# 10XGenomics/lariat

Measured on AMD Instinct MI355X. Metric: read-pairs/sec aligned to hg38 (per-barcode align loop: SMEM seeding + SW + RFA/MAPQ on device); synthetic hg38-scale reference, higher is better.
Workload: dtype u64/i32 (FM-index + integer DP), f64 (RFA scores)

## Files before the change

lariat_amd/csrc/k_rfa.h:

```cpp
#pragma once
#include "k_aln.h"

struct DInf {
    uint8_t *active, *is_proper, *bwa_pick, *active_molecule, *duplicate;
    int32_t *molecule_id, *mapq;
    double *mol_diff, *mol_conf, *sum_move;
    i64* mate;
    int32_t* cand_read;
    i64 *active_idx, *second_best_idx, *split_idx;
    double *second_best_score, *as_score, *split_second_best, *split_score;
    int32_t* split_mapq;
};

#ifdef LH_EMU
static const u64 lh_go_cooked[607] = {
#include "go_rng_cooked.inc"
};
static const uint32_t lh_go_lpow[1848] = {
#include "go_rng_lehmer_pow.inc"
};
#else
__device__ const u64 lh_go_cooked[607] = {
#include "go_rng_cooked.inc"
};
// ... 97 lines not shown
    i64 cs = -1, ce = -1;
    if (R.rid[a] >= 0 && cen_start[R.rid[a]] >= 0) { cs = cen_start[R.rid[a]]; ce = cen_end[R.rid[a]]; }
    return R.pos[a] > cs && R.pos[a] <= ce;
}

struct RfaTab {
    int32_t* plist;
    int32_t* molraw;
    int32_t* mstart;
    int32_t* newid;
    int32_t* nreads;
    double* sval;
    int32_t* seen_rid;
    int32_t* ccnt;
    int32_t* coff;
    int32_t* kidx;
    int32_t* molc;
    int32_t* ppos;
    int32_t* rdl;
    int32_t* firstf;
    int32_t* actc;
    int32_t* psum;
    int32_t* seg0;
    int32_t* seg1;
    int32_t* nbest;
    int32_t* aoff;
    int32_t* alen;
    int32_t* act_store;
    int32_t* act_cand;
    int32_t* act_slot;
    int32_t* tdel;
    int32_t* tset;
    int32_t* mflag;
    double* P;
    u64 *dk0, *dk1, *dk2, *dk3;
    int32_t* htab;
    int32_t* gstk;
    i64* spl;
    int32_t* bestT;
};
template <typename I> struct RfaHot {
    I *nbest, *aoff, *alen, *mflag;
    I *act_store;
    I *act_cand, *act_slot, *tdel, *tset;
    double* P;
};
#ifndef LH_RFA_SM_NR
#define LH_RFA_SM_NR 256
#endif
#ifndef LH_RFA_SM_NC
#define LH_RFA_SM_NC 512
#endif
#ifndef LH_RFA_SM_M
#define LH_RFA_SM_M 128
#endif
static_assert(LH_RFA_SM_NR < 32768 && LH_RFA_SM_NC < 32768 && LH_RFA_SM_M < 32768 && LH_RFA_SM_NR % 4 == 0 && LH_RFA_SM_NC % 4 == 0 && LH_RFA_SM_M % 4 == 0, "the small instance's tables are signed 16-bit words, each array 8-byte aligned");
template <int SMALL> struct RfaHotWord { typedef int32_t type; };
template <> struct RfaHotWord<1> { typedef int16_t type; };
#define RFA_HOT_OFF (16 * LH_RFA_SRC_CHUNK)
#define RFA_HOT_BYTES (8 * LH_RFA_SM_M + 2 * (4 * LH_RFA_SM_M + LH_RFA_SM_NC + 4 * LH_RFA_SM_NR))
#define RFA_T_MASK 0x3fffffff
#define RFA_T_PAIR 0x40000000

__device__ __forceinline__ int dev_mol_active(int alen, int nbest, int change) {
    double active = (double)(alen + change), potential = (double)nbest;
    if (active <= 4) return 0;
    if (active / potential < 0.1) return 0;
    return 1;
}

#define LH_SPLIT_MAX 64
#ifndef LH_RFA_SORT_LDS
#define LH_RFA_SORT_LDS 768
#endif
#define LH_RFA_LDS_BYTES (LH_RFA_SORT_LDS * 12)

static_assert(LH_RFA_LDS_BYTES >= LH_MAPQ_TOP * 64 * (int)sizeof(double), "estimateMapQualities keeps a read's top-15 scores per lane in lds_raw (top[k * 64 + lane])");
#define LH_RFA_NCONT_LDS 1024
#define LH_RFA_SRC_CHUNK 256
static_assert(RFA_HOT_OFF + RFA_HOT_BYTES <= LH_RFA_LDS_BYTES && LH_RFA_SM_NR <= LH_RFA_SRC_CHUNK && LH_RFA_SM_NC <= LH_RFA_SORT_LDS,
              "the small instance: hot tables behind the staging of a whole source (at most a barcode's reads), every contig list sorted in LDS");
#ifndef LH_RFA_MOL_LDS_MIN
#ifndef LH_RFA_TIE_LDS
#define LH_RFA_TIE_LDS (LH_RFA_LDS_BYTES / 4 < 4096 ? LH_RFA_LDS_BYTES / 4 : 4096)
#endif
#ifndef LH_RFA_NET_BLOCK
#define LH_RFA_NET_BLOCK 1024
#endif
static_assert(LH_RFA_NET_BLOCK >= 64 && (LH_RFA_NET_BLOCK & (LH_RFA_NET_BLOCK - 1)) == 0 && LH_RFA_NET_BLOCK * 8 <= LH_RFA_LDS_BYTES, "the network's block lives in lds_raw");
#define LH_RFA_MOL_LDS_MIN 24
#endif

template <typename HOT>
__device__ __forceinline__ double dev_fast_score_w(const DCand& R, const DInf& S, const RfaTab& T, const HOT& H, i64 c_lo, int r0, int M, int src, int snk, double lup,
                                                   int32_t* sLr, int32_t* sFl, double* sLap, int* num_out, int record, int* nmove, int staged = 0) {
    const int lane = LANE();
    double change = 0, alignment_change = 0;
    int num = 0, nm = 0;
    const int n = H.alen[src], ao = H.aoff[src];
    const int reuse = staged && n <= LH_RFA_SRC_CHUNK;
    for (int cb = 0; cb < n; cb += LH_RFA_SRC_CHUNK) {
        int cn = n - cb < LH_RFA_SRC_CHUNK ? n - cb : LH_RFA_SRC_CHUNK;
        if (!reuse) {
            EMU_SYNC();
            for (int s = lane; s < cn; s += 64) {
                int a = H.act_store[ao + cb + s];
                int lr = S.cand_read[c_lo + a] - r0;
                int sm = H.act_cand[lr ^ 1];
                int hm = sm >= 0 && S.molecule_id[c_lo + sm] == src;
                int hp = hm && dev_is_pair(R, c_lo + a, c_lo + sm);
                sLr[s] = lr; sFl[s] = hm | hp << 1; sLap[s] = R.lap[c_lo + a];
            }
            WAVE_SYNC();
        }
        if (snk >= 0) {
            for (int s0 = 0; s0 < cn; s0 += 4) {
                int tq4[4];
                double lap4[4];
#pragma unroll
                for (int u = 0; u < 4; ++u) tq4[u] = s0 + u < cn ? T.bestT[(size_t)sLr[s0 + u] * M + snk] : -1;
#pragma unroll
                for (int u = 0; u < 4; ++u) lap4[u] = tq4[u] >= 0 ? R.lap[c_lo + (tq4[u] & RFA_T_MASK)] : 0.0;
#pragma unroll
                for (int u = 0; u < 4; ++u) {
                    const int tq = tq4[u], s = s0 + u;
                    if (tq >= 0) {
                        int t = tq & RFA_T_MASK, fl = sFl[s];
                        int hm = fl & 1, hp = fl >> 1;
                        int skp = (tq & RFA_T_PAIR) && hm;
                        if (!hp || (hm && skp)) {
                            if (record) { H.tdel[nm] = sLr[s]; H.tset[nm] = t; }
                            nm++;
                        }
                        alignment_change += lap4[u] - sLap[s];
                        if (hp && !skp) alignment_change += lup / 2.0;
                        else if (!hp && skp) alignment_change -= lup / 2.0;
                        num++;
                    }
                }
            }
        }
    }
    if (snk >= 0) {
        int sb = dev_mol_active(H.alen[src], H.nbest[src], 0), sa = dev_mol_active(H.alen[src], H.nbest[src], -num);
        if (!sa && sb) change -= (double)H.nbest[src] * -0.5;
        int kb = dev_mol_active(H.alen[snk], H.nbest[snk], 0), ka = dev_mol_active(H.alen[snk], H.nbest[snk], num);
        if (ka && !kb) change += (double)H.nbest[snk] * -0.5;
        if (H.alen[src] - num == 0 && num > 0) change -= -3.0;
        if (H.alen[snk] == 0 && num > 0) change += -3.0;
        change += alignment_change;
    }
    *num_out = num;
    if (nmove) *nmove = nm;
    return change;
}

__device__ __forceinline__ u64 dev_mix64(u64 x) {
    x ^= x >> 33; x *= 0xff51afd7ed558ccdull; x ^= x >> 33; x *= 0xc4ceb9fe1a85ec53ull; x ^= x >> 33;
    return x;
}

__device__ __forceinline__ void dev_tag_pair_serial(const DCand& R, const DInf& S, double improper, u64 seed, int p, int nA, int nM, u64* ring) {
    const int ra = 2 * p, rb = 2 * p + 1;
    DGoRng rng;
    dev_go_seed(rng, seed, ring);
    double best = -1.7976931348623157e308;
    i64 ba = -1, bm = -1;
    for (i64 a = R.cand_off[ra]; a < R.cand_off[ra + 1]; ++a) {
        if (!R.in_filtered[a]) continue;
        for (i64 m = R.cand_off[rb]; m < R.cand_off[rb + 1]; ++m) {
            if (!R.in_filtered[m]) continue;
            double total = dev_score_aln(R, S, improper, a, m, 0.0) + (dev_go_f64(rng) / 2.0);
            if (total > best) { best = total; ba = a; bm = m; }
        }
    }
    S.active[ba] = 1; S.bwa_pick[ba] = 1;
    if (dev_is_pair(R, ba, bm)) { S.is_proper[ba] = 1; S.is_proper[bm] = 1; }
    S.active[bm] = 1; S.bwa_pick[bm] = 1;
    (void)nA; (void)nM;
}
#ifndef LH_RFA_TAG_WAVE
#define LH_RFA_TAG_WAVE 128
#define LH_RFA_MAPQ_WAVE 128
#define LH_RFA_MQ_CHUNK 384
#endif
static_assert(24 * LH_RFA_MQ_CHUNK <= LH_RFA_LDS_BYTES, "mate staging of estimateMapQualities");


__global__ void __launch_bounds__(256) k_rfa_init(int n_reads, DCand R, DInf S, i64 cand_cap) {
    const i64 n_cand = R.cand_off[n_reads] < cand_cap ? R.cand_off[n_reads] : cand_cap;
    for (i64 g = (i64)blockIdx.x * blockDim.x + threadIdx.x; g < n_cand; g += (i64)gridDim.x * blockDim.x) {
        S.active[g] = 0; S.is_proper[g] = 0; S.bwa_pick[g] = 0; S.active_molecule[g] = 0; S.duplicate[g] = 0; S.molecule_id[g] = -1; S.mapq[g] = 0;
        S.mol_diff[g] = 0; S.mol_conf[g] = 0.00075 * 0.025; S.sum_move[g] = 1.0; S.mate[g] = -1;
    }
    for (i64 r = (i64)blockIdx.x * blockDim.x + threadIdx.x; r < n_reads; r += (i64)gridDim.x * blockDim.x) {
        S.active_idx[r] = -1; S.second_best_idx[r] = -1; S.split_idx[r] = -1; S.second_best_score[r] = 0; S.as_score[r] = 0;
        S.split_second_best[r] = 0; S.split_score[r] = 0; S.split_mapq[r] = 0;
    }
}
__global__ void __launch_bounds__(256) k_rfa_tag(DOpts o, int n_pairs, const u64* __restrict__ name_seed, DCand R, DInf S, i64 cand_cap, int32_t* __restrict__ hp_list,
                                                  int32_t* __restrict__ hp_count) {
    static_assert(LH_RFA_TAG_WAVE <= LH_GO_FAST_DRAWS, "a light pair's draws come from the state-free generator");
    const int p = blockIdx.x * blockDim.x + threadIdx.x, lane = LANE();
    int hv = 0;
    if (p < n_pairs && R.cand_off[2 * p + 2] <= cand_cap) {
        for (int h = 0; h < 2; ++h) {
            const i64 c0 = R.cand_off[2 * p + h];
            if (R.cand_off[2 * p + h + 1] - c0 == 1 && S.cand_read[c0] < 0) S.cand_read[c0] = 2 * p + h;
        }
        int nA = 0, nM = 0;
        for (i64 a = R.cand_off[2 * p]; a < R.cand_off[2 * p + 1]; ++a) nA += R.in_filtered[a] != 0;
        for (i64 m = R.cand_off[2 * p + 1]; m < R.cand_off[2 * p + 2]; ++m) nM += R.in_filtered[m] != 0;
        hv = (i64)nA * nM > LH_RFA_TAG_WAVE;
        if (!hv) dev_tag_pair_serial(R, S, o.improper_pair_penalty, name_seed[p], p, nA, nM, (u64*)nullptr);
    }
    const u64 mh = __ballot(hv);
    if (mh) {
        int basep = 0;
        if (lane == 0) basep = atomicAdd(hp_count, (int32_t)__popcll(mh));
        basep = wave_readlane(basep, 0);
        if (hv) hp_list[basep + lanes_below(mh, lane)] = p;
    }
}
__global__ void __launch_bounds__(64) k_rfa_tag_w(DOpts o, const u64* __restrict__ name_seed, DCand R, DInf S, uint8_t* __restrict__ slab_pool, i64 slab_bytes,
                                                   const int32_t* __restrict__ hp_list, const int32_t* __restrict__ hp_count, int32_t* __restrict__ status) {
    __shared__ __attribute__((aligned(16))) uint8_t lds_raw[8 * 1024];
    const int lane = LANE();
    uint8_t* slab = slab_pool + (size_t)blockIdx.x * (size_t)slab_bytes;
    const double improper = o.improper_pair_penalty;
    const int n_items = *hp_count;
    for (int item = blockIdx.x; item < n_items; item += gridDim.x) {
            const int p = hp_list[item];
            WAVE_SYNC();
            if ((size_t)(R.cand_off[2 * p + 2] - R.cand_off[2 * p]) * 12 + 16 > (size_t)slab_bytes || LH_GO_RING_BYTES > (size_t)slab_bytes) {
                if (lane == 0) status[2 * p] |= LH_ST_POOL_OVERFLOW;
                continue;
            }
            const i64 c_lo = R.cand_off[2 * p];
            const i64 a0 = R.cand_off[2 * p], a1 = R.cand_off[2 * p + 1], m1 = R.cand_off[2 * p + 2];
            int32_t* const fa = (int32_t*)slab;
            double* const fs = (double*)(slab + (((size_t)(m1 - a0) * 4 + 7) & ~(size_t)7));
            int nA = 0, nM = 0;
            for (int side = 0; side < 2; ++side) {
                const i64 lo = side ? a1 : a0, hi = side ? m1 : a1;
                int cnt = 0;
                for (i64 cb = lo; cb < hi; cb += 64) {
                    const i64 c = cb + lane;
                    const int ok = c < hi && R.in_filtered[c];
                    const u64 mk = __ballot(ok);
                    if (ok) {
                        double sc = (double)(R.mismatches[c] * -2 + R.indels[c] * -3);
                        if (R.soft_clipped[c] > 0) { sc -= 5.0 * (double)R.soft_clipped[c]; sc -= (double)R.soft_clipped_length[c] * 0.5; }
                        const int at = nA + cnt + lanes_below(mk, lane);
                        fa[at] = (int32_t)(c - c_lo); fs[at] = sc;
                    }
                    cnt += __popcll(mk);
                }
                if (side) nM = cnt; else nA = cnt;
            }
            WAVE_SYNC();
            u64* const xb = (u64*)lds_raw;
            i64 sd = (i64)name_seed[p] % 2147483647ll;
            if (sd < 0) sd += 2147483647ll;
            if (sd == 0) sd = 89482311;
            const uint32_t x0 = (uint32_t)sd;
            const i64 K = (i64)nA * nM;
            double best = -1.7976931348623157e308;
            i64 bk = 0x7fffffffffffffffll;
            int redraw = 0;
            for (i64 k0 = 0; k0 < K; k0 += 64) {
                const i64 k = k0 + lane, n = k + 1;
                const u64 va = n > LH_GO_LEN ? xb[(n - LH_GO_LEN) & 1023] : dev_go_vec0(x0, (int)(n <= 334 ? 334 - n : 941 - n));
                const u64 vb = n > LH_GO_TAP ? xb[(n - LH_GO_TAP) & 1023] : dev_go_vec0(x0, (int)(LH_GO_LEN - n));
                const u64 x = va + vb;
                xb[n & 1023] = x;
                if (k < K) {
                    const double f = (double)(i64)(x & 0x7fffffffffffffffull) * (1.0 / 9223372036854775808.0);
                    redraw |= f == 1.0;
                    const int ia = (int)(k / nM), im = (int)(k - (i64)ia * nM);
                    const i64 a = c_lo + fa[ia], m = c_lo + fa[nA + im];
                    double t = fs[ia] + fs[nA + im];
                    if (!dev_is_pair(R, a, m)) t += improper;
                    t += 0.0;
                    const double total = t + f / 2.0;
                    if (total > best) { best = total; bk = k; }
                }
                WAVE_SYNC();
            }
            if (__any(redraw)) {
                if (lane == 0) dev_tag_pair_serial(R, S, improper, name_seed[p], p, nA, nM, (u64*)slab + lane);
                WAVE_SYNC();
                continue;
            }
            for (int msk = 32; msk >= 1; msk >>= 1) {
                const double ob = __shfl_xor(best, msk);
                const i64 ok = shfl_xor_i64(bk, msk);
                if (ob > best || (ob == best && ok < bk)) { best = ob; bk = ok; }
            }
            if (lane == 0) {
                const i64 ba = c_lo + fa[(int)(bk / nM)], bm = c_lo + fa[nA + (int)(bk % nM)];
                S.active[ba] = 1; S.bwa_pick[ba] = 1;
                if (dev_is_pair(R, ba, bm)) { S.is_proper[ba] = 1; S.is_proper[bm] = 1; }
                S.active[bm] = 1; S.bwa_pick[bm] = 1;
            }
            WAVE_SYNC();
    }
// ... 600 lines not shown
                                    if (t0 > 0) { best = T.sval[i]; found = T.psum[i]; first = T.firstf[i]; }
                                    scan_tile(A, lr, lrm, arev, 0, tn, t0, e, bp, bi, first);
                                    if (bp != S2_NONE || bi != S2_NONE) { found = 1; const double x = best_of(bp, bi); if (x > best) best = x; }
                                    if (t0 + tn >= msz) { T.sval[i] = found ? best : R.lap[c_lo + T.plist[i]]; T.firstf[i] = first; }
                                    else { T.sval[i] = best; T.psum[i] = found; T.firstf[i] = first; }
                                }
                            }
                        }
                        i0 += msz;
                        continue;
                    }
                    int i1 = NCf;
                    if (i0 + ME_CAP < NCf) i1 = T.mstart[T.molraw[i0 + ME_CAP]];
                    const int tn = i1 - i0;
                    WAVE_SYNC();
                    for (int j = lane; j < tn; j += 64) { const MEnt E = load_ent(i0 + j); me[j] = E; mrd[j] = (uint16_t)(E.rd & 0xffffu); }
                    WAVE_SYNC();
                    RFA_PROF(17)
                    for (int e0 = 0; e0 < tn; e0 += 64) {
                        const int e = e0 + lane;
                        if (e < tn) {
                            const int i = i0 + e, m = T.molraw[i];
                            const int j0 = T.mstart[m] - i0, j1 = T.mstart[m + 1] - i0;
                            const MEnt A = me[e];
                            const int lr = (int)(A.rd & 0x7fffffffu), lrm = lr ^ 1, arev = (int)(A.rd >> 31);
                            int first = 1, bp = S2_NONE, bi = S2_NONE;
                            scan_tile(A, lr, lrm, arev, j0, j1, 0, e, bp, bi, first);
                            T.sval[i] = bp != S2_NONE || bi != S2_NONE ? best_of(bp, bi) : R.lap[c_lo + T.plist[i]];
                            T.firstf[i] = first;
                        }
                    }
                    RFA_PROF(18)
                    i0 = i1;
                }
                WAVE_SYNC();
            }
            int nfirst = 0, nactive = 0;
            for (int base = 0; base < NCf; base += 64) {
                int i = base + lane, first = 0, isact = 0;
                const int pre = i < NCf ? T.firstf[i] : -1;
                if (i < NCf && pre >= 0) { first = pre; isact = S.active[c_lo + T.plist[i]] != 0; }
                u64 mf = __ballot(first), ma = __ballot(isact);
                if (i < NCf) { T.psum[i] = nfirst + lanes_below(mf, lane); T.actc[i] = nactive + lanes_below(ma, lane); }
                nfirst += __popcll(mf); nactive += __popcll(ma);
            }
            if (lane == 0) { T.psum[NCf] = nfirst; T.actc[NCf] = nactive; }
            WAVE_SYNC();
            RFA_PROF(5)
            RFA_FENCE()
            int ao = 0;
            for (int base = 0; base < Mraw; base += 64) {
                int m = base + lane;
                int keep = m < Mraw && T.actc[T.mstart[m + 1]] - T.actc[T.mstart[m]] > 0;
                int nr = keep ? T.psum[T.mstart[m + 1]] - T.psum[T.mstart[m]] : 0;
                u64 mk = __ballot(keep);
                int id = M + lanes_below(mk, lane);
                int inc = wave_scan_add_i32(nr);
                if (keep) {
                    T.newid[m] = id; T.seg0[id] = T.mstart[m]; T.seg1[id] = T.mstart[m + 1];
                    if (!SMALL || id < LH_RFA_SM_M) { H.nbest[id] = nr; H.aoff[id] = ao + inc - nr; H.alen[id] = 0; }
                }
                else if (m < Mraw) T.newid[m] = -1;
                M += __popcll(mk);
                ao += wave_readlane(inc, 63);
            }
            WAVE_SYNC();
            if (SMALL && M > LH_RFA_SM_M) RFA_OVERFLOW()
            if ((size_t)M * (size_t)nR > best_cap) RFA_OVERFLOW()
            for (size_t x = lane; x < (size_t)M * nR; x += 64) T.bestT[x] = -1;
            for (int r = lane; r < nR; r += 64) { H.act_cand[r] = -1; H.act_slot[r] = -1; T.dk0[r] = 0; }
            for (int i = lane; i < NCf; i += 64) S.molecule_id[c_lo + T.plist[i]] = T.newid[T.molraw[i]];
            WAVE_SYNC();
            int nact = 0;
            for (int base = 0; base < NCf; base += 64) {
                int i = base + lane;
                int m = -1, isf = 0, act = -1;
                if (i < NCf) { m = T.newid[T.molraw[i]]; isf = T.firstf[i] && m >= 0; }
                if (isf) {
                    int mr = T.molraw[i], g = r0 + T.rdl[i];
                    double best = -1.7976931348623157e308;
                    int bi = -1, bpos = 0x7fffffff, apos = -1;
                    const i64 cb0 = R.cand_off[g], cb1 = R.cand_off[g + 1];
                    for (i64 b4 = cb0; b4 < cb1; b4 += 4) {
                        int mm[4], pj[4], ac[4];
                        double sv4[4];
#pragma unroll
                        for (int u = 0; u < 4; ++u) {
                            const int ok = b4 + u < cb1;
                            const int lb = (int)(b4 + u - c_lo);
                            mm[u] = ok ? T.molc[lb] : -2; pj[u] = ok ? T.ppos[lb] : 0; ac[u] = ok ? (int)S.active[b4 + u] : 0;
                        }
#pragma unroll
                        for (int u = 0; u < 4; ++u) sv4[u] = mm[u] == mr ? T.sval[pj[u]] : 0.0;
#pragma unroll
                        for (int u = 0; u < 4; ++u) {
                            if (mm[u] != mr) continue;
                            const int lb = (int)(b4 + u - c_lo), j = pj[u];
                            const double sv = sv4[u];
                            if (sv > best || (sv == best && j < bpos)) { best = sv; bi = lb; bpos = j; }
                            if (ac[u] && j > apos) { apos = j; act = lb; }
                        }
                    }
                    T.bestT[(size_t)T.rdl[i] * M + m] = bi;
                    atomicOr((unsigned long long*)&T.dk0[T.rdl[i]], 1ull << ((m >> 6) & 63));
                }
                int hasact = isf && act >= 0;
                u64 mk = __ballot(hasact);
                if (i < NCf) { T.actc[i] = hasact ? act : -1; T.psum[i] = nact + lanes_below(mk, lane); }
                nact += __popcll(mk);
            }
            if (lane == 0) T.psum[NCf] = nact;
            WAVE_SYNC();
            for (int i = lane; i < NCf; i += 64) {
                int m = T.newid[T.molraw[i]];
                if (m < 0 || !T.firstf[i]) continue;
                int lr = T.rdl[i];
                int t = T.bestT[(size_t)lr * M + m] & RFA_T_MASK, tm = T.bestT[(size_t)(lr ^ 1) * M + m];
                if (tm >= 0 && dev_is_pair(R, c_lo + t, c_lo + (tm & RFA_T_MASK))) T.bestT[(size_t)lr * M + m] = t | RFA_T_PAIR;
                int act = T.actc[i];
                if (act >= 0) {
                    int slot = T.psum[i] - T.psum[T.seg0[m]];
                    H.act_store[H.aoff[m] + slot] = act; H.act_cand[lr] = act; H.act_slot[lr] = slot;
                }
            }
            for (int m = lane; m < M; m += 64) H.alen[m] = T.psum[T.seg1[m]] - T.psum[T.seg0[m]];
            WAVE_SYNC();
            for (int m = lane; m < M; m += 64) {
                int diffs = 0;
                for (int k = 0; k < H.alen[m]; ++k) diffs += R.mismatches[c_lo + H.act_store[H.aoff[m] + k]];
                double diff = (double)diffs / (double)H.alen[m];
                for (int k = 0; k < H.alen[m]; ++k) S.mol_diff[c_lo + H.act_store[H.aoff[m] + k]] = diff;
            }
            WAVE_SYNC();
            RFA_PROF(6)
            RFA_FENCE()
            auto stage_source = [&](int src) -> u64 {
                if (M <= 64 || H.alen[src] > LH_RFA_SRC_CHUNK) return ~0ull;
                int num;
                dev_fast_score_w(R, S, T, H, c_lo, r0, M, src, -1, improper, sLr, sFl, sLap, &num, 0, (int*)0);
                u64 mine = 0;
                for (int k = lane; k < H.alen[src]; k += 64) mine |= T.dk0[sLr[k]];
                u64 all = 0;
                for (int b = 0; b < 64 && b * 64 < M; ++b)
                    if (__ballot((int)(mine >> b & 1))) all |= 1ull << b;
                if (M > 64 * 64) all = ~0ull;
                return all;
            };
            int source = 0, idle = 0;
            for (int it = 0; it < 8 * M && idle < M; ++it) {
                ++idle;
                if (H.alen[source] == 0) { source = (source + 1) % M; continue; }
                double bs = -1.7976931348623157e308;
                int bl = -1, bi = 0x7fffffff;
                const u64 groups = stage_source(source);
                const int staged = groups != ~0ull;
                for (int sb = 0; sb < M; sb += 64) {
                    if (!(groups >> ((sb >> 6) & 63) & 1)) continue;
                    int i = sb + lane, num;
                    int snk = (i < M && i != source) ? i : -1;
                    double sc = dev_fast_score_w(R, S, T, H, c_lo, r0, M, source, snk, improper, sLr, sFl, sLap, &num, 0, (int*)0, staged);
                    if (snk >= 0 && num > 0 && (sc > bs || (sc == bs && H.alen[i] > bl))) { bs = sc; bl = H.alen[i]; bi = i; }
                }
                for (int msk = 32; msk >= 1; msk >>= 1) {
                    double os = __shfl_xor(bs, msk);
                    int ol = __shfl_xor(bl, msk), oi = __shfl_xor(bi, msk);
                    int take = oi != 0x7fffffff && (bi == 0x7fffffff || os > bs || (os == bs && (ol > bl || (ol == bl && oi < bi))));
                    if (take) { bs = os; bl = ol; bi = oi; }
                }
                if (bi != 0x7fffffff && (bs > 0 || (bs == 0 && bl > H.alen[source]))) {
                    int num, nmv;
                    dev_fast_score_w(R, S, T, H, c_lo, r0, M, source, bi, improper, sLr, sFl, sLap, &num, lane == 0, &nmv, staged);
                    WAVE_SYNC();
                    idle = 0;
                    if (lane == 0) {
                        for (int k = 0; k < nmv; ++k) {
                            int lr = H.tdel[k], t = H.tset[k];
                            int a = H.act_cand[lr], slot = H.act_slot[lr];
                            int last = H.alen[source] - 1;
                            if (H.alen[source] > 1) {
                                int mv = H.act_store[H.aoff[source] + last];
                                H.act_store[H.aoff[source] + slot] = mv;
                                H.act_slot[S.cand_read[c_lo + mv] - r0] = slot;
                            }
                            H.alen[source] = last;
                            H.act_store[H.aoff[bi] + H.alen[bi]] = t;
                            H.act_slot[lr] = H.alen[bi]; H.act_cand[lr] = t;
                            H.alen[bi]++;
                            S.active[c_lo + a] = 0; S.active[c_lo + t] = 1;
                        }
                    }
                }
                WAVE_SYNC();
                source = (source + 1) % M;
            }
            RFA_PROF(7)
            RFA_FENCE()
            for (int s = 0; s < M; ++s) {
                const u64 groups = stage_source(s);
                const int staged = groups != ~0ull;
                for (int sb = 0; sb < M; sb += 64) {
                    if (!(groups >> ((sb >> 6) & 63) & 1)) continue;
                    int t = sb + lane, num;
                    double sc = dev_fast_score_w(R, S, T, H, c_lo, r0, M, s, (t < M && t != s) ? t : -1, improper, sLr, sFl, sLap, &num, 0, (int*)0, staged);
                    if (t < M) H.P[t] = t == s ? 0.0 : pow(10.0, sc);
                }
                WAVE_SYNC();
                RFA_PROF(8)
                for (int k = lane; k < H.alen[s]; k += 64) {
                    int a = H.act_store[H.aoff[s] + k], lr = S.cand_read[c_lo + a] - r0;
                    double sum = S.sum_move[c_lo + a];
                    const u64 mine = M > 64 && M <= 64 * 64 ? T.dk0[lr] : ~0ull;
                    for (int t0 = 0; t0 < M; t0 += 8) {
                        if (!(mine >> ((t0 >> 6) & 63) & 1)) { t0 = (t0 | 63) - 7; continue; }
                        int q8[8];
#pragma unroll
                        for (int u = 0; u < 8; ++u) q8[u] = t0 + u < M ? T.bestT[(size_t)lr * M + t0 + u] : -1;
#pragma unroll
                        for (int u = 0; u < 8; ++u)
                            if (t0 + u != s && q8[u] >= 0) sum += H.P[t0 + u];
                    }
                    S.sum_move[c_lo + a] = sum;
                }
                WAVE_SYNC();
                RFA_PROF(2)
            }
            RFA_PROF(8)
            RFA_FENCE()
            for (int m = lane; m < M; m += 64) {
                double conf = (double)H.alen[m] / (double)H.nbest[m];
                int soft = 0, diffs = 0;
                for (int k = 0; k < H.alen[m]; ++k) {
                    int a = H.act_store[H.aoff[m] + k];
                    if (R.soft_clipped[c_lo + a] > 0) soft++;
                    diffs += R.mismatches[c_lo + a];
                }
                double diff = (double)diffs / (double)H.alen[m];
                for (int k = 0; k < H.alen[m]; ++k) {
                    int a = H.act_store[H.aoff[m] + k];
                    S.mol_conf[c_lo + a] = conf; S.mol_diff[c_lo + a] = diff;
                }
                H.mflag[m] = (H.alen[m] - soft > 4 && conf > 0.1) ? 1 : 0;
            }
            WAVE_SYNC();
            for (int i = lane; i < NCf; i += 64) {
                int a = T.plist[i], m = S.molecule_id[c_lo + a];
                if (m != -1) S.active_molecule[c_lo + a] = (uint8_t)H.mflag[m];
            }
            WAVE_SYNC();
        }
        {
            double part = 0.0;
            if (do_rfa && M > 0) {
                for (int m = 0; m < M; ++m) {
                    const int al = H.alen[m], ao = H.aoff[m];
                    if (H.mflag[m]) {
                        i64 smallest = 0x7fffffffffffffffll, biggest = -1;
                        for (int k = lane; k < al; k += 64) {
                            i64 p = R.pos[c_lo + H.act_store[ao + k]];
                            if (p > biggest) biggest = p;
                            if (p < smallest) smallest = p;
                        }
                        for (int msk = 32; msk >= 1; msk >>= 1) {
                            const i64 ob = shfl_xor_i64(biggest, msk), os = shfl_xor_i64(smallest, msk);
                            if (ob > biggest) biggest = ob;
                            if (os < smallest) smallest = os;
                        }
                        if (lane == 0 && biggest >= smallest) part += (double)(biggest - smallest) + 1000.0;
                    } else {
                        for (int k = lane; k < al; k += 64) {
                            i64 g = c_lo + H.act_store[ao + k];
                            part += (double)(R.aend[g] - R.pos[g]) * 2.0;
                        }
                    }
                }
            }
            for (int msk = 32; msk >= 1; msk >>= 1) part += __shfl_xor(part, msk);
            if (lane == 0) shd[0] = (do_rfa && M > 0) ? log10((1000.0 + part) / o.genome_length * 0.05) : 0.0;
        }
        WAVE_SYNC();
        double lmp = shd[0];
        RFA_PROF(9)
        RFA_FENCE()
        for (int r = lane; r < nR; r += 64) {
            i64 act = -1;
            for (i64 a = R.cand_off[r0 + r]; a < R.cand_off[r0 + r + 1]; ++a) if (R.in_filtered[a] && S.active[a]) act = a;
            S.active_idx[r0 + r] = act;
        }
        WAVE_SYNC();
        for (int r = lane; r < nR; r += 64) {
            i64 a = S.active_idx[r0 + r], m = S.active_idx[r0 + (r ^ 1)];
            S.mate[a] = m;
        }
        WAVE_SYNC();
        if (lane == 0) bc_lmp[bc] = lmp;
        for (int rb_ = 0; rb_ < nR; rb_ += 64) {
            const int r = rb_ + lane;
            int hv = 0;
            if (r < nR) hv = (R.cand_off[r0 + r + 1] - R.cand_off[r0 + r]) * (R.cand_off[r0 + (r ^ 1) + 1] - R.cand_off[r0 + (r ^ 1)]) > LH_RFA_MAPQ_WAVE;
            const u64 mh = __ballot(hv);
            if (mh) {
                int basep = 0;
                if (lane == 0) basep = atomicAdd(hr_count, (int32_t)__popcll(mh));
                basep = wave_readlane(basep, 0);
                if (hv) { const int at = basep + lanes_below(mh, lane); hr_list[2 * at] = r0 + r; hr_list[2 * at + 1] = bc; }
            }
        }
        WAVE_SYNC();
        RFA_PROF(10)
        RFA_FENCE()
        for (int r = lane; r < nR; r += 64) {
            int gr = r0 + r, gm = r0 + (r ^ 1);
            i64 a0 = R.cand_off[gr], a1 = R.cand_off[gr + 1], m0 = R.cand_off[gm], m1 = R.cand_off[gm + 1];
            if ((a1 - a0) * (m1 - m0) > LH_RFA_MAPQ_WAVE) continue;
            double* const top = (double*)lds_raw;
#define TOPV(k_) top[(k_) * 64 + lane]
            int ntop = 0;
#define TOP_PUSH(v_)                                                                   \
    {                                                                                  \
        double v = (v_);                                                               \
        int k_ = ntop < LH_MAPQ_TOP ? ntop : LH_MAPQ_TOP;                              \
        if (ntop < LH_MAPQ_TOP || v > TOPV(LH_MAPQ_TOP - 1)) {                         \
            if (ntop < LH_MAPQ_TOP) ntop++; else k_ = LH_MAPQ_TOP - 1;                 \
            while (k_ > 0 && TOPV(k_ - 1) < v) { TOPV(k_) = TOPV(k_ - 1); k_--; }      \
            TOPV(k_) = v;                                                              \
        }                                                                              \
    }
            i64 first = -1;
            for (i64 a = a0; a < a1; ++a) if (R.in_filtered[a]) { first = a; break; }
            double bestSingle = -1.7976931348623157e308;
            for (i64 m = m0; m < m1; ++m) {
                if (!R.in_filtered[m]) continue;
                double s = dev_score_aln(R, S, improper, -1, m, lmp);
                if (s > bestSingle) bestSingle = s;
            }
            double pseudo = bestSingle + dev_pseudo_score(R, first, lmp);
            TOP_PUSH(pseudo)
            for (i64 a = a0; a < a1; ++a) {
                if (!R.in_filtered[a]) continue;
                double best = -1.7976931348623157e308;
                for (i64 m = m0; m < m1; ++m) {
                    if (!R.in_filtered[m]) continue;
                    double s = dev_score_aln(R, S, improper, a, m, lmp);
                    if (s > best) best = s;
                }
                TOP_PUSH(best)
            }
            double sb_raw = pseudo, sb_lp = -1000.0;
            i64 sb_aln = -1;
            for (i64 a = a0; a < a1; ++a) {
                if (!R.in_filtered[a] || S.active[a]) continue;
                for (i64 m = m0; m < m1; ++m) {
                    if (!R.in_filtered[m]) continue;
                    double s = dev_score_aln(R, S, improper, a, m, lmp);
                    if (s > sb_lp) { sb_lp = s; sb_raw = dev_score_aln(R, S, improper, a, m, 0.0); sb_aln = a; S.mate[a] = m; }
                }
            }
            i64 act = S.active_idx[gr];
            S.second_best_idx[gr] = sb_aln; S.second_best_score[gr] = sb_raw;
            S.as_score[gr] = dev_score_aln(R, S, improper, act, S.mate[act], 0.0);
            double total = 0;
            for (int k = 0; k < ntop; ++k) total += dev_mapq_pow10(TOPV(k));
            for (i64 a = a0; a < a1; ++a) {
                if (!R.in_filtered[a]) continue;
                S.mapq[a] = dev_mapq(dev_score_aln(R, S, improper, a, S.mate[a], lmp), total, S.sum_move[a], dev_in_centromere(R, cen_start, cen_end, a));
            }
#undef TOP_PUSH
#undef TOPV
        }
        WAVE_SYNC();
        RFA_PROF(11)
        RFA_FENCE()
#ifdef LH_RA_HIST
        if (lane == 0) {
            const unsigned long long dt_ = (unsigned long long)wall_clock64() - bc_t0_;
            int b_ = 0;
            while (b_ < 31 && (dt_ >> (b_ + 1))) ++b_;
            atomicAdd(&lh_rfa_hist[b_], 1ull);
            atomicMax(&lh_rfa_hist[32], dt_);
            atomicAdd(&lh_rfa_hist[33], dt_);
            atomicAdd(&lh_rfa_hist[34], (unsigned long long)NC); atomicAdd(&lh_rfa_hist[35], (unsigned long long)NCf); atomicAdd(&lh_rfa_hist[36], (unsigned long long)M);
// ... 247 lines not shown
```

Before: 55.54 million.

## Spread RFA move scoring and molecule stats across lane groups for small molecule counts

For small barcodes (SMALL template, M<=32), the per-source move scoring now assigns a group of lanes to each sink and splits that source's active reads across the group. Contributions are combined with ballots and shuffles, replacing one lane per sink looping over every read. The molecule confidence and diff pass is parallelised the same way, with lanes splitting each molecule's reads and reducing by shuffle. This is meant to fix poor lane utilisation when M is much smaller than the wavefront width, at the cost of more ballot and shuffle traffic and a serial per-group accumulation loop.

```diff
diff --git a/lariat_amd/csrc/k_rfa.h b/lariat_amd/csrc/k_rfa.h
--- a/lariat_amd/csrc/k_rfa.h
+++ b/lariat_amd/csrc/k_rfa.h
@@ -273,6 +273,82 @@
     }
     *num_out = num;
     if (nmove) *nmove = nm;
+    return change;
+}
+
+template <typename HOT>
+__device__ __forceinline__ double dev_fast_score_spread(const DCand& R, const DInf& S, const RfaTab& T, const HOT& H, i64 c_lo, int r0, int M, int src, double lup,
+                                                        int32_t* sLr, int32_t* sFl, double* sLap, int* num_out, int* snk_out, int* own_out) {
+    const int lane = LANE();
+    int lg = 5;
+    while (lg > 1 && (64 >> lg) < M) --lg;
+    const int G = 1 << lg, sub = lane & (G - 1), base = lane - sub, si = lane >> lg;
+    const int snk = (si < M && si != src) ? si : -1;
+    const uint32_t gmask = 0xffffffffu >> (32 - G);
+    const int n = H.alen[src];
+    int num = 0;
+    dev_fast_score_w(R, S, T, H, c_lo, r0, M, src, -1, lup, sLr, sFl, sLap, &num, 0, (int*)0);
+#ifdef LH_RFA_SPREAD_WEAK
+    const int cn = n - n % (4 * G);
+#else
+    const int cn = n;
+#endif
+    double change = 0, alignment_change = 0;
+    for (int s0 = 0; s0 < cn; s0 += 4 * G) {
+        int tq4[4];
+        double d4[4];
+#pragma unroll
+        for (int u = 0; u < 4; ++u) {
+            const int s = s0 + u * G + sub;
+            tq4[u] = snk >= 0 && s < cn ? T.bestT[(size_t)sLr[s] * M + snk] : -1;
+        }
+#pragma unroll
+        for (int u = 0; u < 4; ++u) d4[u] = tq4[u] >= 0 ? R.lap[c_lo + (tq4[u] & RFA_T_MASK)] : 0.0;
+        int pk = 0;
+#pragma unroll
+        for (int u = 0; u < 4; ++u) {
+            const int tq = tq4[u], s = s0 + u * G + sub;
+            if (tq >= 0) {
+                int fl = sFl[s];
+                int hm = fl & 1, hp = fl >> 1;
+                int skp = (tq & RFA_T_PAIR) && hm;
+                pk |= (4 | (hp && !skp ? 1 : (!hp && skp ? 2 : 0))) << (4 * u);
+                d4[u] = d4[u] - sLap[s];
+            }
+        }
+#pragma unroll
+        for (int u = 0; u < 4; ++u) {
+            const int pu = pk >> (4 * u);
+            const u64 mv = __ballot(pu & 4);
+            if (!mv) continue;
+            const u64 mpl = __ballot((pu & 3) == 1), mmi = __ballot((pu & 3) == 2);
+            const uint32_t gv = (uint32_t)(mv >> base) & gmask, gp = (uint32_t)(mpl >> base) & gmask, gn = (uint32_t)(mmi >> base) & gmask;
+            u64 any = mv;
+            for (int w = G; w < 64; w <<= 1) any |= any >> w;
+            for (uint32_t js = (uint32_t)any & gmask; js; js &= js - 1) {
+                const int j = __builtin_ctz(js);
+                const double d = __shfl(d4[u], base + j);
+                if (gv >> j & 1) {
+                    alignment_change += d;
+                    if (gp >> j & 1) alignment_change += lup / 2.0;
+                    else if (gn >> j & 1) alignment_change -= lup / 2.0;
+                    num++;
+                }
+            }
+        }
+    }
+    if (snk >= 0) {
+        int sb = dev_mol_active(H.alen[src], H.nbest[src], 0), sa = dev_mol_active(H.alen[src], H.nbest[src], -num);
+        if (!sa && sb) change -= (double)H.nbest[src] * -0.5;
+        int kb = dev_mol_active(H.alen[snk], H.nbest[snk], 0), ka = dev_mol_active(H.alen[snk], H.nbest[snk], num);
+        if (ka && !kb) change += (double)H.nbest[snk] * -0.5;
+        if (H.alen[src] - num == 0 && num > 0) change -= -3.0;
+        if (H.alen[snk] == 0 && num > 0) change += -3.0;
+        change += alignment_change;
+    }
+    *num_out = num;
+    *snk_out = snk;
+    if (own_out) *own_out = sub == 0 && si < M ? si : -1;
     return change;
 }
 
@@ -1179,14 +1255,23 @@
                 if (H.alen[source] == 0) { source = (source + 1) % M; continue; }
                 double bs = -1.7976931348623157e308;
                 int bl = -1, bi = 0x7fffffff;
+                int staged = 0;
+                if (SMALL && M <= 32) {
+                    if constexpr (SMALL) {
+                        int num, snk;
+                        double sc = dev_fast_score_spread(R, S, T, H, c_lo, r0, M, source, improper, sLr, sFl, sLap, &num, &snk, (int*)0);
+                        if (snk >= 0 && num > 0) { bs = sc; bl = H.alen[snk]; bi = snk; }
+                    }
+                } else {
                 const u64 groups = stage_source(source);
-                const int staged = groups != ~0ull;
+                staged = groups != ~0ull;
                 for (int sb = 0; sb < M; sb += 64) {
                     if (!(groups >> ((sb >> 6) & 63) & 1)) continue;
                     int i = sb + lane, num;
                     int snk = (i < M && i != source) ? i : -1;
                     double sc = dev_fast_score_w(R, S, T, H, c_lo, r0, M, source, snk, improper, sLr, sFl, sLap, &num, 0, (int*)0, staged);
                     if (snk >= 0 && num > 0 && (sc > bs || (sc == bs && H.alen[i] > bl))) { bs = sc; bl = H.alen[i]; bi = i; }
+                }
                 }
                 for (int msk = 32; msk >= 1; msk >>= 1) {
                     double os = __shfl_xor(bs, msk);
@@ -1223,6 +1308,14 @@
             RFA_PROF(7)
             RFA_FENCE()
             for (int s = 0; s < M; ++s) {
+                if (SMALL && M <= 32) {
+                    if constexpr (SMALL) {
+                        int num, snk, t;
+                        double sc = dev_fast_score_spread(R, S, T, H, c_lo, r0, M, s, improper, sLr, sFl, sLap, &num, &snk, &t);
+                        const double pv = pow(10.0, sc);
+                        if (t >= 0) H.P[t] = t == s ? 0.0 : pv;
+                    }
+                } else {
                 const u64 groups = stage_source(s);
                 const int staged = groups != ~0ull;
                 for (int sb = 0; sb < M; sb += 64) {
@@ -1230,6 +1323,7 @@
                     int t = sb + lane, num;
                     double sc = dev_fast_score_w(R, S, T, H, c_lo, r0, M, s, (t < M && t != s) ? t : -1, improper, sLr, sFl, sLap, &num, 0, (int*)0, staged);
                     if (t < M) H.P[t] = t == s ? 0.0 : pow(10.0, sc);
+                }
                 }
                 WAVE_SYNC();
                 RFA_PROF(8)
@@ -1253,6 +1347,38 @@
             }
             RFA_PROF(8)
             RFA_FENCE()
+            if constexpr (SMALL) {
+                int lgm = 6;
+                while (lgm > 0 && (64 >> lgm) < M) --lgm;
+                const int Gm = 1 << lgm, sub = lane & (Gm - 1);
+                for (int mb = 0; mb < M; mb += 64 >> lgm) {
+                    const int m = mb + (lane >> lgm);
+                    const int al = m < M ? H.alen[m] : 0, ao = m < M ? H.aoff[m] : 0;
+                    int soft = 0, diffs = 0;
+                    for (int k = sub; k < al; k += 4 * Gm) {
+                        int a4[4], sc4[4], mm4[4];
+#pragma unroll
+                        for (int u = 0; u < 4; ++u) a4[u] = k + u * Gm < al ? H.act_store[ao + k + u * Gm] : -1;
+#pragma unroll
+                        for (int u = 0; u < 4; ++u) {
+                            sc4[u] = a4[u] >= 0 ? R.soft_clipped[c_lo + a4[u]] : 0;
+                            mm4[u] = a4[u] >= 0 ? R.mismatches[c_lo + a4[u]] : 0;
+                        }
+#pragma unroll
+                        for (int u = 0; u < 4; ++u) { soft += sc4[u] > 0; diffs += mm4[u]; }
+                    }
+                    for (int msk = Gm >> 1; msk >= 1; msk >>= 1) { soft += __shfl_xor(soft, msk); diffs += __shfl_xor(diffs, msk); }
+                    if (m < M) {
+                        double conf = (double)al / (double)H.nbest[m];
+                        double diff = (double)diffs / (double)al;
+                        for (int k = sub; k < al; k += Gm) {
+                            int a = H.act_store[ao + k];
+                            S.mol_conf[c_lo + a] = conf; S.mol_diff[c_lo + a] = diff;
+                        }
+                        if (sub == 0) H.mflag[m] = (al - soft > 4 && conf > 0.1) ? 1 : 0;
+                    }
+                }
+            } else
             for (int m = lane; m < M; m += 64) {
                 double conf = (double)H.alen[m] / (double)H.nbest[m];
                 int soft = 0, diffs = 0;
```

New measurement: 56.42 million, median of 6. 1.6% higher.
